# florasion/D-VQVAE

Measured on AMD Instinct MI355X. Metric: grasps/sec at batch=65536, N=1024 pts, K=512, higher is better.
Workload: dtype f32 (GEMMs: every fp32 operand as two fp16 pieces, a1 = fp16(a), a2 = fp16((a - a1) * 2^11), weights pre-scaled by one power of two per output row; the 3 partial products a1 b1, a1 b2, a2 b1 are exact in fp32 and accumulate in TWO fp32 accumulators (large / cross terms) on v_mfma_f32_16x16x32_f16; d

## Files before the change

d-vqvae_amd/csrc/pointnet_filter.hip:

```cpp
#include "dvq_internal.h"
#include "pn_filter.h"
#include <vector>

namespace {

typedef __bf16 qbf16x8 __attribute__((ext_vector_type(8)));
typedef _Float16 qf16x8 __attribute__((ext_vector_type(8)));
typedef _Float16 qf16x2 __attribute__((ext_vector_type(2)));
typedef float qf32x2 __attribute__((ext_vector_type(2)));

constexpr float C_ID = 5.0e-5f;
constexpr float DELTA = 1.0e-6f;
constexpr float NEG_BIG = -3.0e38f;

constexpr int F_STAGE2 = 2 * 64 * 128;
constexpr int IMG_OFF_TI = 1024 * 256, IMG_OFF_WN = IMG_OFF_TI + 4096, IMG_OFF_RN = IMG_OFF_WN + 4096;
constexpr int IMG_OFF_W2 = IMG_OFF_RN + 4096, IMG_OFF_K2 = IMG_OFF_W2 + 2 * 128 * 128, IMG_BYTES = IMG_OFF_K2 + 512;
constexpr int F_STAGE3 = 64 * 256;
constexpr int F_OFF_TB = 2 * F_STAGE3;
constexpr int F_SLOT = 4 * 2 * 2 * 2 * 64;
constexpr int F_OFF_W1 = F_OFF_TB + 8 * 4 * 4 * 64 * 4;
constexpr int F_OFF_B1 = F_OFF_W1 + 64 * 4 * 4;
constexpr int F_OFF_B2 = F_OFF_B1 + 64 * 4;
constexpr int F_OFF_K2 = F_OFF_B2 + 128 * 4;
constexpr int F_OFF_SC = F_OFF_K2 + 128 * 4;
constexpr int F_OFF_TI = F_OFF_SC + 64;
constexpr int F_OFF_CS = F_OFF_TI + 4096;
constexpr int F_OFF_WS = F_OFF_CS + 512;
constexpr int F_OFF_E2 = F_OFF_WS + 64;
constexpr int F_LDS = F_OFF_E2 + 4096;
constexpr int F_LDS_TAIL = F_LDS + 3 * 4096 + 4 * 512;
static_assert(F_OFF_W1 >= 2 * F_STAGE2, "the conv3 stages and the triple buffer cover the W2 region");

__device__ __forceinline__ float max_nc(float a, float b) { return __builtin_amdgcn_fmed3f(a, b, 3.0e38f); }
__device__ __forceinline__ float min_nc(float a, float b) { return __builtin_amdgcn_fmed3f(a, b, NEG_BIG); }

__device__ __forceinline__ void q_split2(const float (&v)[8], float s, qf16x8& p1, qf16x8& p2) {
    unsigned hb[4], lb[4];
#pragma unroll
    for (int j = 0; j < 4; ++j) {
        const float a0 = v[2 * j], a1 = v[2 * j + 1];
        asm("v_fma_mixlo_f16 %0, %1, %2, 0 op_sel:[0,0,0] op_sel_hi:[0,0,0]" : "=v"(hb[j]) : "v"(a0), "v"(s));
        asm("v_fma_mixhi_f16 %0, %1, %2, 0 op_sel:[0,0,0] op_sel_hi:[0,0,0]" : "+v"(hb[j]) : "v"(a1), "v"(s));
        asm("v_fma_mixlo_f16 %0, %1, %2, -%3 op_sel:[0,0,0] op_sel_hi:[0,0,1]" : "=v"(lb[j]) : "v"(a0), "v"(s), "v"(hb[j]));
        asm("v_fma_mixhi_f16 %0, %1, %2, -%3 op_sel:[0,0,1] op_sel_hi:[0,0,1]" : "+v"(lb[j]) : "v"(a1), "v"(s), "v"(hb[j]));
    }
    p1 = __builtin_bit_cast(qf16x8, uint4{hb[0], hb[1], hb[2], hb[3]});
    p2 = __builtin_bit_cast(qf16x8, uint4{lb[0], lb[1], lb[2], lb[3]});
}

__device__ __forceinline__ void w2_issue(const uint16_t* __restrict__ planes, int row0, char* stage, int wave, int lane) {
#pragma unroll
    for (int i = 0; i < 4; ++i) {
        const int id = wave * 4 + i;
        const int pl = id >> 3, rb = id & 7;
        const int row = rb * 8 + (lane >> 3);
        const uint16_t* src = planes + pl * (128L * 64) + (long)(row0 + row) * 64 + 8 * ((lane & 7) ^ ((row >> 1) & 7));
        __builtin_amdgcn_global_load_lds((const __attribute__((address_space(1))) void*)src,
                                         (__attribute__((address_space(3))) void*)(stage + (pl * 64 + rb * 8) * 128), 16, 0, 0);
    }
}
__device__ __forceinline__ qf16x8 w2_frag(const char* stage, int pl, int row, int chunk) {
    return *reinterpret_cast<const qf16x8*>(stage + (pl * 64 + row) * 128 + 16 * (chunk ^ ((row >> 1) & 7)));
}

struct W3Regs { uint4 a, b, c, d; };
__device__ __forceinline__ const uint4* w3_src(const char* __restrict__ w3h, int ch0, int wave, int lane, int i) {
    const char* base = w3h + (long)(ch0 + (wave * 4 + i) * 4) * 256;
    const unsigned off = (unsigned)(lane >> 4) * 256u + 16u * (unsigned)(lane & 15);
    return reinterpret_cast<const uint4*>(base + off);
}
__device__ __forceinline__ W3Regs w3_load(const char* __restrict__ w3h, int ch0, int wave, int lane) {
    W3Regs v;
    v.a = *w3_src(w3h, ch0, wave, lane, 0);
    v.b = *w3_src(w3h, ch0, wave, lane, 1);
    v.c = *w3_src(w3h, ch0, wave, lane, 2);
    v.d = *w3_src(w3h, ch0, wave, lane, 3);
    return v;
}
__device__ __forceinline__ uint4* w3_dst(char* stage, int wave, int lane, int i) {
    const int row = (wave * 4 + i) * 4 + (lane >> 4);
    return reinterpret_cast<uint4*>(stage + row * 256 + 16 * ((lane & 15) ^ (row & 15)));
}
__device__ __forceinline__ void w3_store(char* stage, int wave, int lane, const W3Regs& v) {
    *w3_dst(stage, wave, lane, 0) = v.a;
    *w3_dst(stage, wave, lane, 1) = v.b;
    *w3_dst(stage, wave, lane, 2) = v.c;
    *w3_dst(stage, wave, lane, 3) = v.d;
}
__device__ __forceinline__ qf16x8 w3_frag(const char* stage, int row, int chunk) {
    return *reinterpret_cast<const qf16x8*>(stage + row * 256 + 16 * (chunk ^ (row & 15)));
}

__device__ __forceinline__ void merge3(float& a1, float& a2, float& a3, float b1, float b2, float b3) {
    const float x = min_nc(a1, b1), y = max_nc(a2, b2), z = min_nc(a2, b2), w = max_nc(a3, b3);
    a1 = max_nc(a1, b1);
    a2 = max_nc(x, y);
    a3 = max_nc(min_nc(x, y), max_nc(z, w));
}

__device__ __forceinline__ float wave_max(float v) {
#pragma unroll
    for (int o = 32; o >= 1; o >>= 1) v = fmaxf(v, __shfl_xor(v, o));
    return v;
}


__device__ __forceinline__ float g_half_sum(float v) {
    const auto r = __builtin_amdgcn_permlane32_swap(__float_as_uint(v), __float_as_uint(v), false, false);
    return __uint_as_float(r[0]) + __uint_as_float(r[1]);
}
__device__ __forceinline__ float g_half_max(float v) {
    const auto r = __builtin_amdgcn_permlane32_swap(__float_as_uint(v), __float_as_uint(v), false, false);
    return fmaxf(__uint_as_float(r[0]), __uint_as_float(r[1]));
}
template <int CTRL>
__device__ __forceinline__ float g_dpp(float v) {
    return __builtin_bit_cast(float, __builtin_amdgcn_update_dpp(0, __builtin_bit_cast(int, v), CTRL, 0xf, 0xf, true));
}
__device__ __forceinline__ float g_wave_max(float v) {
    v = fmaxf(v, g_dpp<0xB1>(v));
    v = fmaxf(v, g_dpp<0x4E>(v));
    v = fmaxf(v, g_dpp<0x141>(v));
    v = fmaxf(v, g_dpp<0x140>(v));
    v = g_half_max(v);
    return fmaxf(__int_as_float(__builtin_amdgcn_readlane(__float_as_int(v), 0)), __int_as_float(__builtin_amdgcn_readlane(__float_as_int(v), 16)));
}
__device__ __forceinline__ float g_wave_sum(float v) {
    v += g_dpp<0xB1>(v);
    v += g_dpp<0x4E>(v);
    v += g_dpp<0x141>(v);
    v += g_dpp<0x140>(v);
    v = g_half_sum(v);
    return __int_as_float(__builtin_amdgcn_readlane(__float_as_int(v), 0)) + __int_as_float(__builtin_amdgcn_readlane(__float_as_int(v), 16));
}
template <int C>
__device__ __forceinline__ void pn_point_in(const float* __restrict__ src, int N, const float* __restrict__ t, float (&x)[4]) {
    float x0 = src[0], x1 = src[N], x2 = src[2L * N];
    const float x3 = (C > 3) ? src[3L * N] : 0.f;
    if (t) {
        const float n0 = fmaf(x2, t[6], fmaf(x1, t[3], x0 * t[0]));
        const float n1 = fmaf(x2, t[7], fmaf(x1, t[4], x0 * t[1]));
        const float n2 = fmaf(x2, t[8], fmaf(x1, t[5], x0 * t[2]));
        x0 = n0; x1 = n1; x2 = n2;
    }
    x[0] = x0; x[1] = x1; x[2] = x2; x[3] = x3;
}

template <int C>
__device__ __forceinline__ void pn_conv1_split(const float (&xin)[4], const float* w1s, const float* b1s, int h_op, qf16x8 (&h1a)[4], qf16x8 (&h1b)[4],
                                               float& r_p_out) {
    float v[4][8];
    float amax = 0.f;
#pragma unroll
    for (int s = 0; s < 4; ++s) {
#pragma unroll
        for (int j = 0; j < 8; ++j) {
            const f32x4 w = *reinterpret_cast<const f32x4*>(w1s + 32 * h_op + 64 * s + 4 * j);
            float a = fmaf(xin[0], w[0], (b1s + 8 * h_op)[16 * s + j]);
            a = fmaf(xin[1], w[1], a);
            a = fmaf(xin[2], w[2], a);
            if constexpr (C > 3) a = fmaf(xin[3], w[3], a);
            v[s][j] = fmaxf(a, 0.f);
        }
#pragma unroll
        for (int j = 0; j < 8; j += 2) amax = fmaxf(fmaxf(amax, v[s][j]), v[s][j + 1]);
    }
    amax = g_half_max(amax);
    float s_p = 1.f, r_p = 1.f;
    {
        const int ex = (int)((__float_as_uint(amax) >> 23) & 255u);
        if (ex > 20 && ex < 235) {
            s_p = __uint_as_float((unsigned)(127 + 15 - (ex - 126)) << 23);
            r_p = __uint_as_float((unsigned)(127 - 15 + (ex - 126)) << 23);
        }
    }
#pragma unroll
    for (int s = 0; s < 4; ++s) q_split2(v[s], s_p, h1a[s], h1b[s]);
    r_p_out = r_p;
}
template <class Frag, class Emit>
__device__ __forceinline__ void pn_conv2_block(const qf16x8 (&h1a)[4], const qf16x8 (&h1b)[4], float r_p, int t4, const float* k2s, const float* b2s,
                                               int h_op, Frag frag, Emit emit) {
    {
        f32x16 acc;
#pragma unroll
        for (int e = 0; e < 16; ++e) acc[e] = 0.f;
        qf16x8 w1f[4];
#pragma unroll
        for (int s = 0; s < 4; ++s) {
            w1f[s] = frag(t4, 0, s);
            const qf16x8 w2f = frag(t4, 1, s);
            acc = __builtin_amdgcn_mfma_f32_32x32x16_f16(w2f, h1a[s], acc, 0, 0, 0);
            acc = __builtin_amdgcn_mfma_f32_32x32x16_f16(w1f[s], h1b[s], acc, 0, 0, 0);
        }
#pragma unroll
        for (int s = 0; s < 4; ++s) acc = __builtin_amdgcn_mfma_f32_32x32x16_f16(w1f[s], h1a[s], acc, 0, 0, 0);
        float o[16];
#pragma unroll
        for (int e = 0; e < 16; ++e) {
            const int ch = 32 * t4 + (e & 3) + 8 * (e >> 2);
            o[e] = fmaxf(fmaf(acc[e] * r_p, (k2s + 4 * h_op)[ch], (b2s + 4 * h_op)[ch]), 0.f);
        }
        emit(t4, o);
    }
}
template <int C, class Frag, class Emit>
__device__ __forceinline__ void pn_conv12_block(const float (&xin)[4], const float* w1s, const float* b1s, const float* k2s, const float* b2s,
                                                int h_op, Frag frag, Emit emit) {
    qf16x8 h1a[4], h1b[4];
    float r_p;
    pn_conv1_split<C>(xin, w1s, b1s, h_op, h1a, h1b, r_p);
#pragma unroll
    for (int t4 = 0; t4 < 4; ++t4) pn_conv2_block(h1a, h1b, r_p, t4, k2s, b2s, h_op, frag, emit);
}
__device__ __forceinline__ void pn_store_row16(float* dst, const float (&o)[16]) {
#pragma unroll
    for (int g = 0; g < 4; ++g) *reinterpret_cast<f32x4*>(dst + 8 * g) = f32x4{o[4 * g], o[4 * g + 1], o[4 * g + 2], o[4 * g + 3]};
}

template <int C, bool TAIL>
__global__ __launch_bounds__(256, 2) void pn_trunk_filter_kernel(const float* __restrict__ pc, const float* __restrict__ trans,
                                                                 int N, int Npad, int tiles, int deal, long B, const float* __restrict__ W1,
                                                                 const float* __restrict__ b1,
                                                                 const float* __restrict__ b2, const char* __restrict__ w3f,
                                                                 float* __restrict__ h2buf, f32x4* __restrict__ part, qf32x2* __restrict__ part2,
                                                                 unsigned* __restrict__ tstat, const float* __restrict__ cbuf,
                                                                 int abl_arg ) {
    const int abl = DVQ_DIAG_ON ? abl_arg : 0;
    extern __shared__ __attribute__((aligned(16))) char fl[];
    float* tb = reinterpret_cast<float*>(fl + F_OFF_TB);
    float* w1s = reinterpret_cast<float*>(fl + F_OFF_W1);
    float* b1s = reinterpret_cast<float*>(fl + F_OFF_B1);
    float* b2s = reinterpret_cast<float*>(fl + F_OFF_B2);
    float* scs = reinterpret_cast<float*>(fl + F_OFF_SC);
    float* tis = reinterpret_cast<float*>(fl + F_OFF_TI);
    float* wst = reinterpret_cast<float*>(fl + F_OFF_WS);
    const int tid = threadIdx.x, lane = tid & 63;
    const int wave = __builtin_amdgcn_readfirstlane(tid >> 6);
    const int r = lane & 31, h = lane >> 5;
    int h_op = h;
    asm("" : "+v"(h_op));
    constexpr int NPB = TAIL ? 1 : 2;
    const long b_raw = TAIL ? (long)blockIdx.x * 4 + wave : (long)(blockIdx.x / deal);
    const bool live = !TAIL || b_raw < B;
    const long b = live ? b_raw : B - 1;
    const int tile = TAIL ? deal : (int)(blockIdx.x % deal);
    const long rec = b * tiles + tile;
    float* cs = reinterpret_cast<float*>(fl + (TAIL ? F_LDS + 3 * 4096 + 512 * wave : F_OFF_CS));
    float* e2s = reinterpret_cast<float*>(fl + F_OFF_E2) + (TAIL ? 1024 * wave : 0);

    const unsigned long long t_start = (abl & PN_ABL_STAMPS) ? __builtin_amdgcn_s_memtime() : 0ull;
    const unsigned long long r_start = (abl & PN_ABL_CLOCK) ? __builtin_amdgcn_s_memrealtime() : 0ull;
    unsigned long long t_a = 0, t_b = 0, t_c = 0;
    const uint16_t* w2pl = reinterpret_cast<const uint16_t*>(w3f + IMG_OFF_W2);
    w2_issue(w2pl, 0, fl, wave, lane);
    w2_issue(w2pl, 64, fl + F_STAGE2, wave, lane);
    float* k2s = reinterpret_cast<float*>(fl + F_OFF_K2);
    if (tid < 128) k2s[tid] = reinterpret_cast<const float*>(w3f + IMG_OFF_K2)[tid];
    w1s[tid] = W1[tid];
    if (tid < 64) b1s[tid] = b1[tid];
    if (tid < 128) b2s[tid] = b2[tid];
    *reinterpret_cast<f32x4*>(tis + 4 * tid) = *reinterpret_cast<const f32x4*>(w3f + IMG_OFF_TI + 16 * tid);
    if (TAIL) { cs[lane] = cbuf[b * 128 + lane]; cs[64 + lane] = cbuf[b * 128 + 64 + lane]; }
    else if (tid < 128) cs[tid] = cbuf[b * 128 + tid];

    float xin[NPB][4];
    int pidx[NPB];
    bool badpt = false;
#pragma unroll
    for (int pb = 0; pb < NPB; ++pb) {
        int p = point_of_slot(tile, TAIL ? r : wave * 64 + pb * 32 + r, deal);
        pidx[pb] = p;
        if (p >= N) p %= N;
        pn_point_in<C>(pc + b * (long)C * N + p, N, trans ? trans + b * 9 : nullptr, xin[pb]);
        const float x0 = xin[pb][0], x1 = xin[pb][1], x2 = xin[pb][2], x3 = xin[pb][3];
        badpt = badpt || !(fabsf(x0) < 3.0e38f) || !(fabsf(x1) < 3.0e38f) || !(fabsf(x2) < 3.0e38f) || !(fabsf(x3) < 3.0e38f);
    }
    dvq_dma_barrier();
    __builtin_amdgcn_s_waitcnt(0x0F70);
    if (abl & PN_ABL_STAMPS) t_a = __builtin_amdgcn_s_memtime();
    float cnorm;
    {
        const float cq = fmaf(cs[lane], cs[lane], cs[64 + lane] * cs[64 + lane]);
        cnorm = sqrtf(g_wave_sum(cq)) * 1.0001f;
    }

// ... 267 lines not shown
            F_INTERLEAVE();
            finish(c, 1, m1, m2);
            F_MFMA_BLOCK(accB, wf[3]);
            F_CHAIN_BLOCK(accA, m1, m2, ctag_c);
            F_INTERLEAVE();
            finish(c, 2, m1, m2);
            F_CHAIN_BLOCK(accB, m1, m2, ctag_c);
            finish(c, 3, m1, m2);
            if (c + 1 < 16) w3_store(fl + (stage ^ 1) * F_STAGE3, wave, lane, wreg);
            stage ^= 1;
        }
    } else {
    f32x4 accP[NRB];
#pragma unroll 1
    for (int c4 = 0; c4 < ((abl & PN_ABL_NO_CONV3) ? 0 : 16); c4 += 4) {
    unsigned ctag4[16];
#pragma unroll
    for (int e = 0; e < 16; ++e) asm("s_or_b32 %0, %1, %2" : "=s"(ctag4[e]) : "s"((unsigned)(((c4 >> 2) & 3) << 5)), "i"(e));
#pragma unroll
    for (int u = 0; u < 4; ++u) {
        const int c = c4 + u;
        const int stage = u & 1;
        const bool pending = u != 0;
        if (!(abl & PN_ABL_NO_CHUNK_BARRIER)) dvq_lds_barrier();
        if (c + 1 < 16 && !(abl & PN_ABL_NO_W3_LOADS)) wreg = w3_load(w3h, 64 * (c + 1), wave, lane);
        if (u == 0 && c > 0 && !(abl & PN_ABL_NO_PUBLISH)) {
            publish(c - 4 + wave);
            dvq_lds_barrier();
        }
        const char* st = fl + stage * F_STAGE3;
        qf16x8 wf[4][4];
#pragma unroll
        for (int cb = 0; cb < 4; ++cb)
#pragma unroll
            for (int ks = 0; ks < 4; ++ks) wf[cb][ks] = w3_frag(st, 16 * cb + l16, 4 * ks + qchunk);
        f32x4 accA[NRB], accB[NRB];
        float m1, m2;
        F_MFMA_BLOCK(accA, wf[0]);
        if (pending) {
            F_CHAIN_BLOCK(accP, m1, m2, ctag4);
            F_INTERLEAVE();
            if (!(abl & PN_ABL_NO_HANDOVER)) finish(c - 1, 3, m1, m2);
            else if (m1 + m2 == 12345.f) tb[lane] = m1;
        }
        F_MFMA_BLOCK(accB, wf[1]);
        F_CHAIN_BLOCK(accA, m1, m2, ctag4);
        F_INTERLEAVE();
        if (!(abl & PN_ABL_NO_HANDOVER)) finish(c, 0, m1, m2);
        else if (m1 + m2 == 12345.f) tb[lane] = m1;
        F_MFMA_BLOCK(accA, wf[2]);
        F_CHAIN_BLOCK(accB, m1, m2, ctag4);
        F_INTERLEAVE();
        if (!(abl & PN_ABL_NO_HANDOVER)) finish(c, 1, m1, m2);
        else if (m1 + m2 == 12345.f) tb[lane] = m1;
        F_MFMA_BLOCK(accP, wf[3]);
        F_CHAIN_BLOCK(accA, m1, m2, ctag4);
        F_INTERLEAVE();
        if (!(abl & PN_ABL_NO_HANDOVER)) finish(c, 2, m1, m2);
        else if (m1 + m2 == 12345.f) tb[lane] = m1;
        if (u == 3) {
            F_CHAIN_BLOCK(accP, m1, m2, ctag4);
            if (!(abl & PN_ABL_NO_HANDOVER)) finish(c, 3, m1, m2);
            else if (m1 + m2 == 12345.f) tb[lane] = m1;
        }
        if (c + 1 < 16 && !(abl & PN_ABL_NO_W3_LOADS)) w3_store(fl + (stage ^ 1) * F_STAGE3, wave, lane, wreg);
    }
    }
    }
#undef F_MFMA_BLOCK
#undef F_CHAIN_BLOCK
#undef F_INTERLEAVE
    dvq_lds_barrier();
    if constexpr (TAIL) {
#pragma unroll 1
        for (int q = 12; q < 16; ++q) publish(q);
    } else if (!(abl & PN_ABL_NO_PUBLISH)) {
        publish(12 + wave);
    }
    if ((abl & PN_ABL_STAMPS) && tid == 0) {
        const unsigned long long t_end = __builtin_amdgcn_s_memtime();
        auto q = [](unsigned long long d) { d >>= 6; return (unsigned)(d > 255 ? 255 : d); };
        tstat[4 * rec + 3] = q(t_a - t_start) | (q(t_b - t_a) << 8) | (q(t_c - t_b) << 16) | (q((t_end - t_c) >> 3) << 24);
        if (abl & PN_ABL_CLOCK) {
            const unsigned long long r_end = __builtin_amdgcn_s_memrealtime();
            tstat[4 * rec + 3] = (unsigned)((t_end - t_start) * 100ull / (r_end - r_start + 1));
        }
    }
}

template <int CTRL>
__device__ __forceinline__ float q_dpp(float v) {
    return __builtin_bit_cast(float, __builtin_amdgcn_update_dpp(0, __builtin_bit_cast(int, v), CTRL, 0xf, 0xf, true));
}
__device__ __forceinline__ float exact_dot_regs(const f32x4& w0, const f32x4& w1, const f32x4& a, const f32x4& c) {
    float s = w0[0] * a[0];
    s = fmaf(w0[1], a[1], s);
    s = fmaf(w0[2], a[2], s);
    s = fmaf(w0[3], a[3], s);
    s = fmaf(w1[0], c[0], s);
    s = fmaf(w1[1], c[1], s);
    s = fmaf(w1[2], c[2], s);
    s = fmaf(w1[3], c[3], s);
    s += q_dpp<0xB1>(s);
    s += q_dpp<0x4E>(s);
    s += q_dpp<0x141>(s);
    s += q_dpp<0x140>(s);
    return s;
}
__device__ __forceinline__ float exact_dot(const f32x4& w0, const f32x4& w1, const float* __restrict__ hrow, int j) {
    return exact_dot_regs(w0, w1, *reinterpret_cast<const f32x4*>(hrow + 4 * j), *reinterpret_cast<const f32x4*>(hrow + 4 * j + 64));
}
__device__ __forceinline__ float max_nan(float a, float b) { return (a != a || b != b) ? __builtin_nanf("") : fmaxf(a, b); }

__device__ __forceinline__ unsigned f2key(float v) {
    const unsigned u = __float_as_uint(v);
    return (u & 0x80000000u) ? ~u : (u | 0x80000000u);
}
__device__ __forceinline__ float key2f(unsigned k) { return __uint_as_float((k & 0x80000000u) ? (k & 0x7fffffffu) : ~k); }

__device__ unsigned long long g_pn_faults[2];

constexpr int PAIR_CAP = 2048;
constexpr int FB_CAP = 512;
constexpr unsigned short NO_ANCHOR = 0xFFFFu;
constexpr int TODO_CAP = 2 * PAIR_CAP;
template <int C>
__global__ __launch_bounds__(256, 4) void pn_exact_kernel(const f32x4* __restrict__ part, const qf32x2* __restrict__ part2, int tiles, int deal,
                                                       float* h2buf , int recompute,
                                                       const float* __restrict__ pc, const float* __restrict__ trans,
                                                       const float* __restrict__ W1, const float* __restrict__ b1, const float* __restrict__ b2,
                                                       const char* __restrict__ w3f,
                                                       int N, int Npad, const float* __restrict__ w3, const float* __restrict__ b3,
                                                       const float* __restrict__ wnorm, const float* __restrict__ rnorm,
                                                       const unsigned* __restrict__ tstat, const float* __restrict__ cbuf, int relu, int exhaustive,
                                                       int pair_cap, int fb_cap, float* __restrict__ feat, long ld_feat,
                                                       unsigned long long* __restrict__ stats, int abl_arg) {
    const int abl = DVQ_DIAG_ON ? abl_arg : 0;
    __shared__ unsigned short anchor[1024];
    __shared__ int pair_list[PAIR_CAP];
    __shared__ int fb_list[FB_CAP];
    __shared__ short all_list[1024];
    __shared__ int pair_count, fb_count, all_count;
    __shared__ float fb_part[4][16];
    __shared__ float hm[PN_MAX_TILES], dm[PN_MAX_TILES], rd[PN_MAX_TILES];
    __shared__ unsigned best_k[1024];
    __shared__ float wcs[1024];
    __shared__ int pcnt[1024];
    __shared__ unsigned sorted[PAIR_CAP];
    __shared__ int wave_tot[4];
    __shared__ unsigned row_mask[32];
    __shared__ unsigned done_mask[PN_MAX_POINTS / 32];
    __shared__ int todo_count;
    __shared__ __attribute__((aligned(16))) float w1s[64 * 4 + 64];
    static_assert(PAIR_CAP >= 1024, "sorted[] holds the 1 024 anchors");
    static_assert(PN_MAX_POINTS <= 65536, "a point fits a 16-bit list entry");
    const int tid = threadIdx.x, g = tid >> 4, j = tid & 15;
    const long b = blockIdx.x;
    if (tid == 0) { pair_count = 0; fb_count = 0; all_count = 0; todo_count = 0; }
    if (tid < 32) row_mask[tid] = 0;
    done_mask[tid] = 0; done_mask[tid + 256] = 0;
    w1s[tid] = W1[tid];
    if (tid < 64) w1s[256 + tid] = b1[tid];
#pragma unroll
    for (int i = 0; i < 4; ++i) pcnt[tid + 256 * i] = 0;
    int nonfinite_point = 0;
    if (tid < tiles) {
        const unsigned* ts = tstat + 4 * (b * tiles + tid);
        hm[tid] = __uint_as_float(ts[0]) * 1.00001f;
        dm[tid] = __uint_as_float(ts[1]) * 1.00001f;
        rd[tid] = __uint_as_float(ts[2]) * 1.00001f;
        nonfinite_point = ts[3] != 0 && !(abl & PN_ABL_STAMPS);
    }
    if (__syncthreads_or(nonfinite_point)) {
        for (int n = tid; n < 1024; n += 256) feat[b * ld_feat + n] = __builtin_nanf("");
        return;
    }
    float* h2 = h2buf + b * (long)Npad * 128;
    const bool wrap_small = Npad <= 2 * N;
    const f32x4* pt = part + b * (long)tiles * 1024;
    const qf32x2* pt2 = part2 + b * (long)tiles * 1024;
    const bool stamps = DVQ_DIAG_ON && stats && (abl & PN_ABL_STAMPS);
    unsigned long long tp[8] = {0, 0, 0, 0, 0, 0, 0, 0};
    if (stamps) tp[0] = __builtin_amdgcn_s_memtime();
    unsigned n_single = 0, n_multi = 0, n_cand = 0, n_wave = 0, n_suspect = 0;
    auto bound_of = [&](float wn, float rn, int t) { return fmaf(rn, dm[t], fmaf(wn, rd[t], fmaf(C_ID * wn, dm[t], 2.0f * DELTA * wn * hm[t]))); };
    struct Scan { float lb, ub, e_all, top_star; int t_star; bool all; };
    auto scan_tiles = [&](int n, float wn, float rn, float top0, float top1, float top2, float top3) {
        Scan s;
        bool nonfinite = false;
        auto fold = [&](int t, float top) {
            const float e = bound_of(wn, rn, t), l = top - e;
            nonfinite = nonfinite || !(e < 3.0e38f) || !(fabsf(top) < 3.0e38f);
            s.e_all = fmaxf(s.e_all, e);
            if (l > s.lb) { s.t_star = t; s.top_star = top; }
            s.lb = fmaxf(s.lb, l);
            s.ub = fmaxf(s.ub, top + e);
        };
        {
            const float e0 = bound_of(wn, rn, 0);
            s.e_all = e0;
            s.lb = top0 - e0;
            s.ub = top0 + e0;
            s.t_star = 0;
            s.top_star = top0;
            nonfinite = !(e0 < 3.0e38f) || !(fabsf(top0) < 3.0e38f);
            if (tiles > 1) fold(1, top1);
            if (tiles > 2) fold(2, top2);
            if (tiles > 3) fold(3, top3);
        }
        for (int t0 = 4; t0 < tiles; t0 += 4) {
            float top[4];
#pragma unroll
            for (int u = 0; u < 4; ++u) top[u] = pt[min(t0 + u, tiles - 1) * 1024 + n][0];
#pragma unroll
            for (int u = 0; u < 4; ++u)
                if (t0 + u < tiles) fold(t0 + u, top[u]);
        }
        s.all = exhaustive || nonfinite || !(s.e_all < 3.0e38f) || !(s.lb > NEG_BIG) || !(s.lb < 3.0e38f);
        return s;
    };
    auto point_of_score = [&](int t, float v) {
        int p = point_of_slot(t, slot_of_id(__float_as_uint(v) & 255u), deal);
        if (p >= N) p = wrap_small ? p - N : p % N;
        if (abl & PN_ABL_FEW_ROWS) p &= 63;
        return p;
    };
    unsigned short* todo = reinterpret_cast<unsigned short*>(pair_list);
    int todo_base = 0;
    auto claim = [&](int p) {
        const unsigned bit = 1u << (p & 31);
        if (atomicOr(&done_mask[p >> 5], bit) & bit) return;
        const int slot = atomicAdd(&todo_count, 1) - todo_base;
        if (slot < TODO_CAP) todo[slot] = (unsigned short)p;
    };
    auto fill_rows = [&](bool all) {
        dvq_lds_barrier();
        const int end = __builtin_amdgcn_readfirstlane(todo_count), listed = end - todo_base;
        todo_base = end;
        const bool forced = listed > TODO_CAP;
        const bool whole = all || forced;
        const int cnt = whole ? N : listed;
        const int lane = tid & 63, r = lane & 31, h = lane >> 5;
        const float* k2g = reinterpret_cast<const float*>(w3f + IMG_OFF_K2);
        const uint16_t* w2pl = reinterpret_cast<const uint16_t*>(w3f + IMG_OFF_W2);
        for (int i0 = 32 * __builtin_amdgcn_readfirstlane(tid >> 6); i0 < cnt; i0 += 128) {
            if (whole && !forced && done_mask[i0 >> 5] == ~0u) continue;
            int h_op = h;
            asm volatile("" : "+v"(h_op));
            const int i = min(i0 + r, cnt - 1);
            const int p = whole ? i : (int)todo[i];
            float x[4];
            pn_point_in<C>(pc + b * (long)C * N + p, N, trans ? trans + b * 9 : nullptr, x);
            float* row = h2 + (long)p * 128 + 4 * h;
            const bool mine = i0 + r < cnt;
            qf16x8 h1a[4], h1b[4];
            float r_p;
            pn_conv1_split<C>(x, w1s, w1s + 256, h_op, h1a, h1b, r_p);
#pragma unroll 1
            for (int t4 = 0; t4 < 4; ++t4)
                pn_conv2_block(h1a, h1b, r_p, t4, k2g, b2, h_op,
                               [&](int t, int pl, int s) { return *reinterpret_cast<const qf16x8*>(w2pl + pl * (128 * 64) + (32 * t + r) * 64 + 8 * (2 * s + h)); },
                               [&](int t, const float (&o)[16]) { if (mine) pn_store_row16(row + 32 * t, o); });
            if (whole && lane == 0) done_mask[i0 >> 5] = ~0u;
            if (stats && lane == 0) {
                atomicAdd(stats + 10, 1ull);
                atomicAdd(stats + 11, (unsigned long long)min(32, cnt - i0));
            }
        }
        asm volatile("s_waitcnt vmcnt(0)" ::: "memory");
        dvq_lds_barrier();
    };
    auto sort_by_point = [&](auto code_at, int count, bool first) {
        for (int i = tid; i < count; i += 256) {
            const unsigned code = code_at(i);
            if (code != ~0u) atomicAdd(&pcnt[(code >> 10) & 1023], 1);
        }
        dvq_lds_barrier();
        const int c0 = pcnt[4 * tid], c1 = pcnt[4 * tid + 1], c2 = pcnt[4 * tid + 2], c3 = pcnt[4 * tid + 3];
        if (stats) {
            const unsigned m = (unsigned)(c0 != 0) | (unsigned)(c1 != 0) << 1 | (unsigned)(c2 != 0) << 2 | (unsigned)(c3 != 0) << 3;
            const int sh = 4 * (tid & 7);
            int rows;
            if (first) { if (m) atomicOr(&row_mask[tid >> 3], m << sh); rows = __popc(m); }
            else rows = __popc(m & ~(row_mask[tid >> 3] >> sh));
            if (rows) atomicAdd(stats + 8, (unsigned long long)rows);
        }
        int incl = c0 + c1 + c2 + c3;
        int lane_op = tid & 63;
        asm volatile("" : "+v"(lane_op));
#pragma unroll
        for (int o = 1; o < 64; o <<= 1) {
            const int v = __builtin_amdgcn_ds_bpermute(4 * (lane_op - o), incl);
            if ((tid & 63) >= o) incl += v;
        }
        if ((tid & 63) == 63) wave_tot[tid >> 6] = incl;
        dvq_lds_barrier();
        int base = 0;
        for (int w = 0; w < (tid >> 6); ++w) base += wave_tot[w];
        const int total = wave_tot[0] + wave_tot[1] + wave_tot[2] + wave_tot[3];
        const int excl = base + incl - (c0 + c1 + c2 + c3);
        pcnt[4 * tid] = excl;
        pcnt[4 * tid + 1] = excl + c0;
        pcnt[4 * tid + 2] = excl + c0 + c1;
        pcnt[4 * tid + 3] = excl + c0 + c1 + c2;
        dvq_lds_barrier();
        for (int i = tid; i < count; i += 256) {
            const unsigned code = code_at(i);
            if (code != ~0u) sorted[atomicAdd(&pcnt[(code >> 10) & 1023], 1)] = code;
        }
        dvq_lds_barrier();
        return total;
    };
    auto dots = [&](int total, bool first) {
        const int per = (total + 15) >> 4, i0 = g * per, i1 = min(total, i0 + per);
        f32x4 cen_a = {0.f, 0.f, 0.f, 0.f}, cen_b = cen_a;
        if (first) { cen_a = *reinterpret_cast<const f32x4*>(cbuf + b * 128 + 4 * j); cen_b = *reinterpret_cast<const f32x4*>(cbuf + b * 128 + 4 * j + 64); }
        for (int i = i0; i < i1; i += 4) {
            f32x4 w0[4], w1[4], ha[4], hb[4];
            int nn[4];
#pragma unroll
            for (int u = 0; u < 4; ++u) {
                const unsigned code = sorted[min(i + u, i1 - 1)];
                nn[u] = (int)(code & 1023u);
                const unsigned woff = (code & 1023u) * 512u + 16u * (unsigned)j, hoff = (code >> 10) * 512u + 16u * (unsigned)j;
                w0[u] = *reinterpret_cast<const f32x4*>(reinterpret_cast<const char*>(w3) + woff);
                w1[u] = *reinterpret_cast<const f32x4*>(reinterpret_cast<const char*>(w3) + woff + 256);
                ha[u] = *reinterpret_cast<const f32x4*>(reinterpret_cast<const char*>(h2) + hoff);
                hb[u] = *reinterpret_cast<const f32x4*>(reinterpret_cast<const char*>(h2) + hoff + 256);
            }
            float v[4], wc[4];
#pragma unroll
            for (int u = 0; u < 4; ++u) {
                v[u] = exact_dot_regs(w0[u], w1[u], ha[u], hb[u]);
                wc[u] = first ? exact_dot_regs(w0[u], w1[u], cen_a, cen_b) : 0.f;
            }
            if (j == 0) {
#pragma unroll
                for (int u = 0; u < 4; ++u)
                    if (i + u < i1) {
                        if (first) { best_k[nn[u]] = f2key(v[u]); wcs[nn[u]] = wc[u]; }
                        else atomicMax(&best_k[nn[u]], f2key(v[u]));
                    }
            }
        }
    };
    {
        float top[4][4], wn[4], rn[4];
#pragma unroll
        for (int ci = 0; ci < 4; ++ci) {
            const int n = tid + 256 * ci;
#pragma unroll
            for (int u = 0; u < 4; ++u) top[ci][u] = pt[min(u, tiles - 1) * 1024 + n][0];
            wn[ci] = wnorm[n]; rn[ci] = rnorm[n];
        }
#pragma unroll
        for (int ci = 0; ci < 4; ++ci) {
            const int n = tid + 256 * ci;
            const Scan s = scan_tiles(n, wn[ci], rn[ci], top[ci][0], top[ci][1], top[ci][2], top[ci][3]);
            best_k[n] = f2key(NEG_BIG);
            wcs[n] = 0.f;
            if (s.all) {
                all_list[atomicAdd(&all_count, 1)] = (short)n;
                anchor[n] = NO_ANCHOR;
            } else
                anchor[n] = (unsigned short)point_of_score(s.t_star, s.top_star);
        }
    }
    dvq_lds_barrier();
    if (stamps) tp[1] = __builtin_amdgcn_s_memtime();
    auto anchor_code = [&](int n) { const unsigned p = anchor[n]; return p == NO_ANCHOR ? ~0u : (unsigned)n | (p << 10); };
    const int n_anchor = sort_by_point(anchor_code, 1024, true);
#pragma unroll
    for (int i = 0; i < 4; ++i) pcnt[tid + 256 * i] = 0;
    if (stamps) tp[2] = __builtin_amdgcn_s_memtime();
    if (recompute) {
        for (int i = tid; i < n_anchor; i += 256) {
            const int p = (int)(sorted[i] >> 10);
            if (i == 0 || (int)(sorted[i - 1] >> 10) != p) claim(p);
        }
        fill_rows(false);
    }
    if (!(abl & PN_ABL_NO_DOTS)) dots(n_anchor, true);
    dvq_lds_barrier();
    if (stamps) tp[3] = __builtin_amdgcn_s_memtime();
    float lo_0 = 1.f, lo_1 = 1.f, lo_2 = 1.f, lo_3 = 1.f, hi_0 = 0.f, hi_1 = 0.f, hi_2 = 0.f, hi_3 = 0.f;
    f32x4 nf0 = pt[tid], nf1 = pt[min(1, tiles - 1) * 1024 + tid], nf2 = pt[min(2, tiles - 1) * 1024 + tid], nf3 = pt[min(3, tiles - 1) * 1024 + tid];
    qf32x2 ng0 = pt2[tid], ng1 = pt2[min(1, tiles - 1) * 1024 + tid], ng2 = pt2[min(2, tiles - 1) * 1024 + tid], ng3 = pt2[min(3, tiles - 1) * 1024 + tid];
    float nwn = wnorm[tid], nrn = rnorm[tid];
#pragma unroll 1
    for (int ci = 0; ci < 4; ++ci) {
        const int n = tid + 256 * ci;
        const float wn = nwn, rn = nrn;
        const f32x4 f0 = nf0, f1 = nf1, f2 = nf2, f3 = nf3;
        const qf32x2 g0 = ng0, g1 = ng1, g2 = ng2, g3 = ng3;
        if (ci < 3) {
            const int nx = n + 256;
            nf0 = pt[nx]; nf1 = pt[min(1, tiles - 1) * 1024 + nx]; nf2 = pt[min(2, tiles - 1) * 1024 + nx]; nf3 = pt[min(3, tiles - 1) * 1024 + nx];
            ng0 = pt2[nx]; ng1 = pt2[min(1, tiles - 1) * 1024 + nx]; ng2 = pt2[min(2, tiles - 1) * 1024 + nx]; ng3 = pt2[min(3, tiles - 1) * 1024 + nx];
            nwn = wnorm[nx]; nrn = rnorm[nx];
        }
        const Scan s = scan_tiles(n, wn, rn, f0[0], f1[0], f2[0], f3[0]);
        if (s.all) continue;
        const float lb = s.lb;
        float L = lb;
        if (!(abl & PN_ABL_NO_RULE2)) {
            const float v1 = key2f(best_k[n]), wc1 = wcs[n];
            L = fmaxf(lb, (v1 - wc1) - 4.0e-7f * (fabsf(v1) + fabsf(wc1)));
        }
        int cands = 1;
        bool whole = false;
        float lo_c = lb, hi_c = s.ub;
        auto consider = [&](int t, const f32x4& q, const qf32x2& q45) {
            const float et = bound_of(wn, rn, t);
            const unsigned suspect = (__float_as_uint(q[3]) >> 16) & 1u;
            n_suspect += suspect;
            if (!suspect && !(q[0] + et >= L)) return;
            unsigned flags = __float_as_uint(q[3]) & 0xFFFFu;
            unsigned forced = suspect ? 0xFFFFu : 0u;
            auto take = [&](float v) {
                const int p = point_of_score(t, v);
                const int slot = atomicAdd(&pair_count, 1);
                if (slot < pair_cap) pair_list[slot] = n | (p << 10);
                else {
                    const unsigned bit = 1u << pn_group_of_id(__float_as_uint(v));
                    flags |= bit;
                    forced |= bit;
                }
                ++cands;
            };
            const float sc5[5] = {q[0], q[1], q[2], q45[0], q45[1]};
#pragma unroll 1
            for (int k = (t == s.t_star ? 1 : 0); k < 5; ++k) {
                const float v = k == 0 ? sc5[0] : k == 1 ? sc5[1] : k == 2 ? sc5[2] : k == 3 ? sc5[3] : sc5[4];
                if (!(v + et >= L)) break;
                take(v);
            }
            while (flags) {
                const int wh = __ffs(flags) - 1;
                flags &= flags - 1;
                if (!((forced >> wh) & 1u) && !(abl & PN_ABL_NO_RULE1)) {
                    auto of_group = [&](float v) { return pn_group_of_id(__float_as_uint(v)) == wh; };
                    const bool m0 = of_group(sc5[0]), m1 = of_group(sc5[1]), m2 = of_group(sc5[2]), m3 = of_group(sc5[3]), m4 = of_group(sc5[4]);
                    const float second = m4 ? sc5[4] : m3 ? sc5[3] : m2 ? sc5[2] : m1 ? sc5[1] : sc5[0];
                    const float u = (int)m0 + (int)m1 + (int)m2 + (int)m3 + (int)m4 >= 2 ? second : sc5[4];
                    if (u + et < L) continue;
                }
                const int slot = atomicAdd(&fb_count, 1);
                if (slot < fb_cap) fb_list[slot] = n | (t << 10) | (wh << 20);
                else if (!whole) {
                    whole = true;
                    all_list[atomicAdd(&all_count, 1)] = (short)n;
                }
                ++n_wave;
            }
        };
        f32x4 q0 = f0, q1 = f1, q2 = f2, q3 = f3;
        qf32x2 h0 = g0, h1 = g1, h2q = g2, h3 = g3;
#pragma unroll 1
        for (int t0 = 0; t0 < tiles; t0 += 4) {
            if (t0 > 0) {
                q0 = pt[min(t0, tiles - 1) * 1024 + n]; q1 = pt[min(t0 + 1, tiles - 1) * 1024 + n];
                q2 = pt[min(t0 + 2, tiles - 1) * 1024 + n]; q3 = pt[min(t0 + 3, tiles - 1) * 1024 + n];
                h0 = pt2[min(t0, tiles - 1) * 1024 + n]; h1 = pt2[min(t0 + 1, tiles - 1) * 1024 + n];
                h2q = pt2[min(t0 + 2, tiles - 1) * 1024 + n]; h3 = pt2[min(t0 + 3, tiles - 1) * 1024 + n];
            }
#pragma unroll 1
            for (int u = 0; u < 4 && t0 + u < tiles; ++u) {
                const f32x4 q = u == 0 ? q0 : u == 1 ? q1 : u == 2 ? q2 : q3;
                const qf32x2 q45 = u == 0 ? h0 : u == 1 ? h1 : u == 2 ? h2q : h3;
                consider(t0 + u, q, q45);
            }
        }
        if (whole) { lo_c = 1.f; hi_c = 0.f; }
        lo_0 = ci == 0 ? lo_c : lo_0; hi_0 = ci == 0 ? hi_c : hi_0;
        lo_1 = ci == 1 ? lo_c : lo_1; hi_1 = ci == 1 ? hi_c : hi_1;
        lo_2 = ci == 2 ? lo_c : lo_2; hi_2 = ci == 2 ? hi_c : hi_2;
        lo_3 = ci == 3 ? lo_c : lo_3; hi_3 = ci == 3 ? hi_c : hi_3;
        n_single += cands == 1;
        n_multi += cands != 1;
        n_cand += cands;
    }
    dvq_lds_barrier();
    if (stamps) tp[4] = __builtin_amdgcn_s_memtime();
    auto eval_all_list = [&](int count) {
        for (int i = 0; i < count; i += 4) {
            f32x4 w0[4], w1[4];
            float best[4];
#pragma unroll
            for (int u = 0; u < 4; ++u) {
                const int n = all_list[min(i + u, count - 1)];
                w0[u] = *reinterpret_cast<const f32x4*>(w3 + n * 128 + 4 * j);
                w1[u] = *reinterpret_cast<const f32x4*>(w3 + n * 128 + 4 * j + 64);
                best[u] = NEG_BIG;
            }
            for (int p = g; p < N; p += 16) {
                const float* hr = reinterpret_cast<const float*>(reinterpret_cast<const char*>(h2) + ((unsigned)p * 512u + 16u * (unsigned)j));
                const f32x4 ha = *reinterpret_cast<const f32x4*>(hr), hb = *reinterpret_cast<const f32x4*>(hr + 64);
#pragma unroll
                for (int u = 0; u < 4; ++u) best[u] = max_nan(best[u], exact_dot_regs(w0[u], w1[u], ha, hb));
                if (best[0] != best[0] && best[1] != best[1] && best[2] != best[2] && best[3] != best[3]) break;
            }
            if (j == 0) {
#pragma unroll
                for (int u = 0; u < 4; ++u) fb_part[u][g] = best[u];
            }
            dvq_lds_barrier();
            if (tid < 4 && i + tid < count) {
                float v = fb_part[tid][0];
                for (int k = 1; k < 16; ++k) v = max_nan(v, fb_part[tid][k]);
                best_k[all_list[i + tid]] = (v != v) ? 0xffffffffu : f2key(v);
            }
            dvq_lds_barrier();
        }
    };
    unsigned n_bad = 0;
    int n_sorted = 0, nfb = 0;
#pragma unroll 1
    for (int pass = 0; pass < 2; ++pass) {
        if (pass == 0) {
            const int npairs = min(pair_count, pair_cap);
            n_sorted = sort_by_point([&](int i) { return (unsigned)pair_list[i]; }, npairs, false);
            if (stamps) tp[5] = __builtin_amdgcn_s_memtime();
            nfb = (abl & PN_ABL_NO_GROUPS) ? 0 : min(fb_count, fb_cap);
            if (recompute && all_count == 0) {
                for (int i = tid; i < n_sorted; i += 256) {
                    const int p = (int)(sorted[i] >> 10);
                    if (i == 0 || (int)(sorted[i - 1] >> 10) != p) claim(p);
                }
                for (int i = tid; i < 16 * nfb; i += 256) {
                    const int code = fb_list[i >> 4];
                    int p = point_of_slot((code >> 10) & 1023, pn_group_slot((code >> 20) & 15, i & 15), deal);
                    if (p >= N) p %= N;
                    claim(p);
                }
            }
        } else {
            dvq_lds_barrier();
            if (tid == 0) all_count = 0;
            dvq_lds_barrier();
#pragma unroll
            for (int ci = 0; ci < 4; ++ci) {
                const int n = tid + 256 * ci;
                const float lo_c = ci == 0 ? lo_0 : ci == 1 ? lo_1 : ci == 2 ? lo_2 : lo_3, hi_c = ci == 0 ? hi_0 : ci == 1 ? hi_1 : ci == 2 ? hi_2 : hi_3;
                if (!(lo_c <= hi_c) || (abl & ~PN_ABL_VALID)) continue;
                const float v = key2f(best_k[n]), wc = wcs[n];
                const float x = v - wc, slack = 4.0e-7f * (fabsf(v) + fabsf(wc));
                if (!(x >= lo_c - slack && x <= hi_c + slack)) {
                    all_list[atomicAdd(&all_count, 1)] = (short)n;
                    ++n_bad;
                }
            }
            dvq_lds_barrier();
        }
        const int n_all = __builtin_amdgcn_readfirstlane(all_count);
        if (recompute && (pass == 0 || n_all > 0)) fill_rows(n_all > 0);
        if (pass == 0) {
            if (!(abl & PN_ABL_NO_DOTS)) dots(n_sorted, false);
            if (stamps) tp[6] = __builtin_amdgcn_s_memtime();
            for (int i = tid >> 6; i < nfb; i += 4) {
                const int code = fb_list[i];
                const int n = code & 1023, t = (code >> 10) & 1023, grp = (code >> 20) & 15;
                const float* wr = reinterpret_cast<const float*>(reinterpret_cast<const char*>(w3) + ((unsigned)n * 512u + 16u * (unsigned)j));
                const f32x4 w0 = *reinterpret_cast<const f32x4*>(wr), w1 = *reinterpret_cast<const f32x4*>(wr + 64);
                float best = NEG_BIG;
                {
                    f32x4 ha[4], hb[4];
#pragma unroll
                    for (int u = 0; u < 4; ++u) {
                        int p = point_of_slot(t, pn_group_slot(grp, 4 * (g & 3) + u), deal);
                        if (p >= N) p %= N;
                        const float* hr = reinterpret_cast<const float*>(reinterpret_cast<const char*>(h2) + ((unsigned)p * 512u + 16u * (unsigned)j));
                        ha[u] = *reinterpret_cast<const f32x4*>(hr);
                        hb[u] = *reinterpret_cast<const f32x4*>(hr + 64);
                    }
#pragma unroll
                    for (int u = 0; u < 4; ++u) best = fmaxf(best, exact_dot_regs(w0, w1, ha[u], hb[u]));
                }
                if (j == 0) atomicMax(&best_k[n], f2key(best));
            }
            dvq_lds_barrier();
        }
        eval_all_list(n_all);
    }
    if (n_suspect) atomicAdd(&g_pn_faults[0], (unsigned long long)n_suspect);
    if (n_bad) atomicAdd(&g_pn_faults[1], (unsigned long long)n_bad);
    int tid_op = tid;
    asm volatile("" : "+v"(tid_op));
#pragma unroll
    for (int i = 0; i < 4; ++i) {
        const int n = tid_op + 256 * i;
        const unsigned k = best_k[n];
        const float v = (k == 0xffffffffu ? __builtin_nanf("") : key2f(k)) + b3[n];
        feat[b * ld_feat + n] = relu ? (v != v ? v : fmaxf(v, 0.f)) : v;
    }
    if (stamps && tid == 0) {
        const unsigned long long t_end = __builtin_amdgcn_s_memtime();
        atomicAdd(stats + 4, (tp[1] - tp[0]) + (tp[4] - tp[3])); atomicAdd(stats + 5, (tp[2] - tp[1]) + (tp[5] - tp[4]));
        atomicAdd(stats + 6, (tp[3] - tp[2]) + (tp[6] - tp[5])); atomicAdd(stats + 7, t_end - tp[6]);
        atomicAdd(stats + 9, tp[3] - tp[0]);
    }
    if (stats) {
        if (n_single) atomicAdd(stats + 0, (unsigned long long)n_single);
        if (n_multi) atomicAdd(stats + 1, (unsigned long long)n_multi);
        if (n_wave) atomicAdd(stats + 2, (unsigned long long)n_wave);
        if (n_cand) atomicAdd(stats + 3, (unsigned long long)n_cand);
    }
}

constexpr int CENTER_SPB = 4;
template <int C>
__global__ __launch_bounds__(256) void pn_center_kernel(const float* __restrict__ pc, const float* __restrict__ trans, int N, long B,
                                                        const float* __restrict__ W1, const float* __restrict__ b1,
                                                        const float* __restrict__ W2, const float* __restrict__ b2,
                                                        float* __restrict__ cbuf, unsigned* __restrict__ tstat, int tiles) {
    __shared__ float w2t[64][129];
    __shared__ float h1c[4][64];
    __shared__ float h2c[4][128];
    const int tid = threadIdx.x, q = tid >> 6, k = tid & 63;
    for (int i = tid; i < 128 * 64; i += 256) w2t[i & 63][i >> 6] = W2[i];
    for (int sb = 0; sb < CENTER_SPB; ++sb) {
        const long b = (long)blockIdx.x * CENTER_SPB + sb;
        if (b >= B) break;
        for (int i = tid; i < 4 * tiles; i += 256) tstat[b * 4 * tiles + i] = 0u;
        {
            const int p = (int)(((long)q * N) / 4);
            const float* src = pc + b * (long)C * N + p;
            float x0 = src[0], x1 = src[N], x2 = src[2L * N];
            const float x3 = (C > 3) ? src[3L * N] : 0.f;
            if (trans) {
                const float* t = trans + b * 9;
                const float n0 = fmaf(x2, t[6], fmaf(x1, t[3], x0 * t[0]));
                const float n1 = fmaf(x2, t[7], fmaf(x1, t[4], x0 * t[1]));
                const float n2 = fmaf(x2, t[8], fmaf(x1, t[5], x0 * t[2]));
                x0 = n0; x1 = n1; x2 = n2;
            }
            const float* w = W1 + 4 * k;
            float a = x0 * w[0];
            a = fmaf(x1, w[1], a);
            a = fmaf(x2, w[2], a);
            a = fmaf(x3, w[3], a);
            h1c[q][k] = fmaxf(a + b1[k], 0.f);
        }
        dvq_lds_barrier();
#pragma unroll
        for (int half = 0; half < 2; ++half) {
            const int ch = k + 64 * half;
            float a = 0.f;
            for (int i = 0; i < 64; ++i) a = fmaf(w2t[i][ch], h1c[q][i], a);
            h2c[q][ch] = fmaxf(a + b2[ch], 0.f);
        }
        dvq_lds_barrier();
        if (tid < 128) cbuf[b * 128 + tid] = 0.25f * ((h2c[0][tid] + h2c[1][tid]) + (h2c[2][tid] + h2c[3][tid]));
    }
}

__global__ __launch_bounds__(256) void pn_filter_pack_kernel(const float* __restrict__ w3, _Float16* __restrict__ wh,
                                                             float* __restrict__ tinv, float* __restrict__ wnorm,
                                                             float* __restrict__ rnorm) {
    const int lane = threadIdx.x & 63;
    const int n = blockIdx.x * 4 + (threadIdx.x >> 6);
    const float a = w3[n * 128 + lane], c = w3[n * 128 + 64 + lane];
    const float amax = wave_max(fmaxf(fabsf(a), fabsf(c)));
    float sq = fmaf(a, a, c * c);
#pragma unroll
    for (int o = 32; o >= 1; o >>= 1) sq += __shfl_xor(sq, o);
    float t = 1.f;
    const int ex = (int)((__float_as_uint(amax) >> 23) & 255u);
    if (ex > 20 && ex < 235) t = __uint_as_float((unsigned)(127 + 15 - (ex - 126)) << 23);
    float rs = 0.f;
#pragma unroll
    for (int half = 0; half < 2; ++half) {
        const int pos = 64 * half + lane;
        const int q = pos & 15;
        const int k = (pos & ~15) + ((q & 3) | ((q & 4) << 1) | ((q & 8) >> 1));
        const float v = w3[n * 128 + k] * t;
        const _Float16 hv = (_Float16)v;
        wh[n * 128 + pos] = hv;
        const float res = v - (float)hv;
        rs = fmaf(res, res, rs);
    }
#pragma unroll
    for (int o = 32; o >= 1; o >>= 1) rs += __shfl_xor(rs, o);
    if (lane == 0) {
        tinv[n] = 1.0f / t;
        wnorm[n] = sqrtf(sq) * 1.00001f;
        rnorm[n] = sqrtf(rs) / t * 1.00001f;
    }
}

__global__ __launch_bounds__(256) void pn_filter_pack_w2_kernel(const float* __restrict__ w2, _Float16* __restrict__ planes,
                                                                float* __restrict__ kinv) {
    const int lane = threadIdx.x & 63;
    const int n = blockIdx.x * 4 + (threadIdx.x >> 6);
    const float v = w2[n * 64 + lane];
    const float amax = wave_max(fabsf(v));
    float t = 1.f;
    const int ex = (int)((__float_as_uint(amax) >> 23) & 255u);
    if (ex > 20 && ex < 235) t = __uint_as_float((unsigned)(127 + 15 - (ex - 126)) << 23);
    const float vs = v * t;
    const _Float16 p1 = (_Float16)vs;
    const _Float16 p2 = (_Float16)(vs - (float)p1);
    planes[n * 64 + lane] = p1;
    planes[128 * 64 + n * 64 + lane] = p2;
    if (lane == 0) kinv[n] = 1.0f / t;
}

}

size_t dvq_pn_filter_image_bytes() { return (size_t)IMG_BYTES; }

int dvq_launch_pn_filter_pack(const float* w2, const float* w3, void* image, hipStream_t st) {
    char* im = (char*)image;
    DVQ_LAUNCH(pn_filter_pack_kernel, dim3(256), dim3(256), 0, st, w3, reinterpret_cast<_Float16*>(im),
               reinterpret_cast<float*>(im + IMG_OFF_TI), reinterpret_cast<float*>(im + IMG_OFF_WN),
               reinterpret_cast<float*>(im + IMG_OFF_RN));
    DVQ_CHECK_LAUNCH("pn_filter_pack");
    DVQ_LAUNCH(pn_filter_pack_w2_kernel, dim3(32), dim3(256), 0, st, w2, reinterpret_cast<_Float16*>(im + IMG_OFF_W2),
               reinterpret_cast<float*>(im + IMG_OFF_K2));
    DVQ_CHECK_LAUNCH("pn_filter_pack_w2");
    return DVQ_OK;
}

static int filter_geometry(int N, PnGeometry* g) {
    *g = pn_geometry(N, dvq_knobs().pn_tail != 0);
    DVQ_REQUIRE(g->tiles <= PN_MAX_TILES, "pointnet: the filtered trunk takes at most %d points", PN_MAX_POINTS);
    return DVQ_OK;
}
#ifdef DVQ_DIAG
static int pn_abl() { const char* e = getenv("DVQ_PN_ABL"); return e ? atoi(e) : 0; }
#else
static constexpr int pn_abl() { return 0; }
#endif

using TrunkFilterKernel = decltype(&pn_trunk_filter_kernel<3, false>);
static TrunkFilterKernel trunk_filter_kernel(int C, bool tail) {
    static const TrunkFilterKernel k[2][2] = {{&pn_trunk_filter_kernel<3, false>, &pn_trunk_filter_kernel<3, true>},
                                              {&pn_trunk_filter_kernel<4, false>, &pn_trunk_filter_kernel<4, true>}};
    return k[C == 4][tail];
}
static decltype(&pn_center_kernel<3>) center_kernel(int C) { return C == 4 ? &pn_center_kernel<4> : &pn_center_kernel<3>; }
static decltype(&pn_exact_kernel<3>) exact_kernel(int C) { return C == 4 ? &pn_exact_kernel<4> : &pn_exact_kernel<3>; }
static bool pn_recompute() { return dvq_knobs().pn_recompute && !dvq_knobs().pn_exhaustive; }

int dvq_launch_pn_filter_front(const PnBatch& in, const PnTrunkWeights& w, const PnSlot& sl, unsigned long long* stats, hipStream_t st) {
    PnGeometry g;
    DVQ_PROPAGATE(filter_geometry(in.N, &g));
    static DvqOncePerDevice attr_once[2][2];
    for (int c = 0; c < 2; ++c)
        for (int tail = 0; tail < 2; ++tail)
            DVQ_PROPAGATE(dvq_lds_limit(attr_once[c][tail], reinterpret_cast<const void*>(trunk_filter_kernel(3 + c, tail)),
                                        tail ? F_LDS_TAIL : (DVQ_DIAG_ON ? 100 * 1024 : F_LDS), "pointnet"));
    const long B = in.B, grid = B * g.deal;
    DVQ_REQUIRE(B * g.tiles < (1L << 31), "pointnet: grid too large");
    if (stats && hipMemsetAsync(stats, 0, PN_STATS_BYTES, st) != hipSuccess) {
        dvq_set_error("pointnet: hipMemsetAsync failed");
        return DVQ_ELAUNCH;
    }
    {
// ... 111 lines not shown
```

Before: 191,300.

## Restructure fill_rows: per-wave output column slice with register-resident W2 and prefetched points

The row-filling loop changes from each wave computing all 128 output channels for its own 32 points to each wave computing one 32-channel slice for every point. This lets the wave keep its W2 fragments in registers for the whole loop instead of reloading them from global memory. The next batch of point coordinates is prefetched while the current batch runs its convolution. The transform matrix and the k2/b2 vectors are hoisted into scalars or LDS, done_mask updates are batched to the end of the loop, and the stats and fault atomics move earlier to shorten live ranges. In exchange, every wave now walks all points, so the conv1 work is repeated across the four waves, and register pressure rises.

```diff
diff --git a/d-vqvae_amd/csrc/pointnet_filter.hip b/d-vqvae_amd/csrc/pointnet_filter.hip
--- a/d-vqvae_amd/csrc/pointnet_filter.hip
+++ b/d-vqvae_amd/csrc/pointnet_filter.hip
@@ -133,6 +133,17 @@
     v += g_dpp<0x140>(v);
     v = g_half_sum(v);
     return __int_as_float(__builtin_amdgcn_readlane(__float_as_int(v), 0)) + __int_as_float(__builtin_amdgcn_readlane(__float_as_int(v), 16));
+}
+template <int C>
+__device__ __forceinline__ void pn_point_raw(const float* __restrict__ src, int N, float (&x)[4]) {
+    x[0] = src[0]; x[1] = src[N]; x[2] = src[2L * N];
+    x[3] = (C > 3) ? src[3L * N] : 0.f;
+}
+__device__ __forceinline__ void pn_point_xform(const float (&t)[9], float (&x)[4]) {
+    const float n0 = fmaf(x[2], t[6], fmaf(x[1], t[3], x[0] * t[0]));
+    const float n1 = fmaf(x[2], t[7], fmaf(x[1], t[4], x[0] * t[1]));
+    const float n2 = fmaf(x[2], t[8], fmaf(x[1], t[5], x[0] * t[2]));
+    x[0] = n0; x[1] = n1; x[2] = n2;
 }
 template <int C>
 __device__ __forceinline__ void pn_point_in(const float* __restrict__ src, int N, const float* __restrict__ t, float (&x)[4]) {
@@ -706,15 +717,18 @@
     __shared__ unsigned done_mask[PN_MAX_POINTS / 32];
     __shared__ int todo_count;
     __shared__ __attribute__((aligned(16))) float w1s[64 * 4 + 64];
+    __shared__ float k2s[128], b2s[128];
     static_assert(PAIR_CAP >= 1024, "sorted[] holds the 1 024 anchors");
     static_assert(PN_MAX_POINTS <= 65536, "a point fits a 16-bit list entry");
-    const int tid = threadIdx.x, g = tid >> 4, j = tid & 15;
+    int tid = threadIdx.x;
+    const int g = tid >> 4, j = tid & 15;
     const long b = blockIdx.x;
     if (tid == 0) { pair_count = 0; fb_count = 0; all_count = 0; todo_count = 0; }
     if (tid < 32) row_mask[tid] = 0;
     done_mask[tid] = 0; done_mask[tid + 256] = 0;
     w1s[tid] = W1[tid];
     if (tid < 64) w1s[256 + tid] = b1[tid];
+    if (tid < 128) { k2s[tid] = reinterpret_cast<const float*>(w3f + IMG_OFF_K2)[tid]; b2s[tid] = b2[tid]; }
 #pragma unroll
     for (int i = 0; i < 4; ++i) pcnt[tid + 256 * i] = 0;
     int nonfinite_point = 0;
@@ -788,41 +802,73 @@
         if (slot < TODO_CAP) todo[slot] = (unsigned short)p;
     };
     auto fill_rows = [&](bool all) {
+        const int lane = tid & 63, r = lane & 31, h = lane >> 5;
+        const int wv = __builtin_amdgcn_readfirstlane(tid >> 6);
+        qf16x8 wf[2][4];
+        {
+            const uint16_t* w2pl = reinterpret_cast<const uint16_t*>(w3f + IMG_OFF_W2) + (32 * wv + r) * 64 + 8 * h;
+#pragma unroll
+            for (int pl = 0; pl < 2; ++pl)
+#pragma unroll
+                for (int s = 0; s < 4; ++s) wf[pl][s] = *reinterpret_cast<const qf16x8*>(w2pl + pl * (128 * 64) + 16 * s);
+        }
+        float tm[9] = {0.f, 0.f, 0.f, 0.f, 0.f, 0.f, 0.f, 0.f, 0.f};
+        if (trans) {
+#pragma unroll
+            for (int k = 0; k < 9; ++k) tm[k] = trans[b * 9 + k];
+        }
         dvq_lds_barrier();
+#pragma unroll
+        for (int s = 0; s < 4; ++s) asm volatile("" : "+v"(wf[0][s]), "+v"(wf[1][s]));
+#pragma unroll
+        for (int k = 0; k < 9; ++k) tm[k] = __int_as_float(__builtin_amdgcn_readfirstlane(__float_as_int(tm[k])));
         const int end = __builtin_amdgcn_readfirstlane(todo_count), listed = end - todo_base;
         todo_base = end;
         const bool forced = listed > TODO_CAP;
         const bool whole = all || forced;
         const int cnt = whole ? N : listed;
-        const int lane = tid & 63, r = lane & 31, h = lane >> 5;
-        const float* k2g = reinterpret_cast<const float*>(w3f + IMG_OFF_K2);
-        const uint16_t* w2pl = reinterpret_cast<const uint16_t*>(w3f + IMG_OFF_W2);
-        for (int i0 = 32 * __builtin_amdgcn_readfirstlane(tid >> 6); i0 < cnt; i0 += 128) {
-            if (whole && !forced && done_mask[i0 >> 5] == ~0u) continue;
+        auto next_batch = [&](int i0) {
+            if (whole && !forced)
+                while (i0 < cnt && __builtin_amdgcn_readfirstlane(done_mask[i0 >> 5]) == ~0u) i0 += 32;
+            return i0;
+        };
+        auto request = [&](int i0, int& p, float (&x)[4]) {
+            const int i = min(i0 + r, cnt - 1);
+            p = whole ? i : (int)todo[i];
+            pn_point_raw<C>(pc + b * (long)C * N + p, N, x);
+        };
+        int i0 = next_batch(0), p_next = 0;
+        float x_next[4] = {0.f, 0.f, 0.f, 0.f};
+        if (i0 < cnt) {
+            request(i0, p_next, x_next);
+            asm volatile("" : "+v"(x_next[0]), "+v"(x_next[1]), "+v"(x_next[2]), "+v"(x_next[3]));
+        }
+        while (i0 < cnt) {
+            const int p = p_next;
+            float x[4] = {x_next[0], x_next[1], x_next[2], x_next[3]};
+            if (trans) pn_point_xform(tm, x);
+            const int i1 = next_batch(i0 + 32);
+            if (i1 < cnt) request(i1, p_next, x_next);
             int h_op = h;
             asm volatile("" : "+v"(h_op));
-            const int i = min(i0 + r, cnt - 1);
-            const int p = whole ? i : (int)todo[i];
-            float x[4];
-            pn_point_in<C>(pc + b * (long)C * N + p, N, trans ? trans + b * 9 : nullptr, x);
-            float* row = h2 + (long)p * 128 + 4 * h;
-            const bool mine = i0 + r < cnt;
+            float* row = reinterpret_cast<float*>(reinterpret_cast<char*>(h2) + ((unsigned)p * 512u + 16u * (unsigned)h));
             qf16x8 h1a[4], h1b[4];
             float r_p;
             pn_conv1_split<C>(x, w1s, w1s + 256, h_op, h1a, h1b, r_p);
-#pragma unroll 1
-            for (int t4 = 0; t4 < 4; ++t4)
-                pn_conv2_block(h1a, h1b, r_p, t4, k2g, b2, h_op,
-                               [&](int t, int pl, int s) { return *reinterpret_cast<const qf16x8*>(w2pl + pl * (128 * 64) + (32 * t + r) * 64 + 8 * (2 * s + h)); },
-                               [&](int t, const float (&o)[16]) { if (mine) pn_store_row16(row + 32 * t, o); });
-            if (whole && lane == 0) done_mask[i0 >> 5] = ~0u;
-            if (stats && lane == 0) {
+            pn_conv2_block(h1a, h1b, r_p, wv, k2s, b2s, h_op,
+                           [&](int, int pl, int s) { return wf[pl][s]; },
+                           [&](int t, const float (&o)[16]) { pn_store_row16(row + 32 * t, o); });
+            if (i1 < cnt) asm volatile("" : "+v"(x_next[0]), "+v"(x_next[1]), "+v"(x_next[2]), "+v"(x_next[3]));
+            if (stats && wv == 0 && lane == 0) {
                 atomicAdd(stats + 10, 1ull);
                 atomicAdd(stats + 11, (unsigned long long)min(32, cnt - i0));
             }
+            i0 = i1;
         }
         asm volatile("s_waitcnt vmcnt(0)" ::: "memory");
         dvq_lds_barrier();
+        if (whole)
+            for (int i = tid; i < (N + 31) >> 5; i += 256) done_mask[i] = ~0u;
     };
     auto sort_by_point = [&](auto code_at, int count, bool first) {
         for (int i = tid; i < count; i += 256) {
@@ -1036,6 +1082,13 @@
     }
     dvq_lds_barrier();
     if (stamps) tp[4] = __builtin_amdgcn_s_memtime();
+    if (n_suspect) atomicAdd(&g_pn_faults[0], (unsigned long long)n_suspect);
+    if (stats) {
+        if (n_single) atomicAdd(stats + 0, (unsigned long long)n_single);
+        if (n_multi) atomicAdd(stats + 1, (unsigned long long)n_multi);
+        if (n_wave) atomicAdd(stats + 2, (unsigned long long)n_wave);
+        if (n_cand) atomicAdd(stats + 3, (unsigned long long)n_cand);
+    }
     auto eval_all_list = [&](int count) {
         for (int i = 0; i < count; i += 4) {
             f32x4 w0[4], w1[4];
@@ -1067,10 +1120,10 @@
             dvq_lds_barrier();
         }
     };
-    unsigned n_bad = 0;
     int n_sorted = 0, nfb = 0;
 #pragma unroll 1
     for (int pass = 0; pass < 2; ++pass) {
+        asm volatile("" : "+v"(tid));
         if (pass == 0) {
             const int npairs = min(pair_count, pair_cap);
             n_sorted = sort_by_point([&](int i) { return (unsigned)pair_list[i]; }, npairs, false);
@@ -1092,6 +1145,7 @@
             dvq_lds_barrier();
             if (tid == 0) all_count = 0;
             dvq_lds_barrier();
+            unsigned n_bad = 0;
 #pragma unroll
             for (int ci = 0; ci < 4; ++ci) {
                 const int n = tid + 256 * ci;
@@ -1104,6 +1158,7 @@
                     ++n_bad;
                 }
             }
+            if (n_bad) atomicAdd(&g_pn_faults[1], (unsigned long long)n_bad);
             dvq_lds_barrier();
         }
         const int n_all = __builtin_amdgcn_readfirstlane(all_count);
@@ -1136,8 +1191,6 @@
         }
         eval_all_list(n_all);
     }
-    if (n_suspect) atomicAdd(&g_pn_faults[0], (unsigned long long)n_suspect);
-    if (n_bad) atomicAdd(&g_pn_faults[1], (unsigned long long)n_bad);
     int tid_op = tid;
     asm volatile("" : "+v"(tid_op));
 #pragma unroll
@@ -1152,12 +1205,6 @@
         atomicAdd(stats + 4, (tp[1] - tp[0]) + (tp[4] - tp[3])); atomicAdd(stats + 5, (tp[2] - tp[1]) + (tp[5] - tp[4]));
         atomicAdd(stats + 6, (tp[3] - tp[2]) + (tp[6] - tp[5])); atomicAdd(stats + 7, t_end - tp[6]);
         atomicAdd(stats + 9, tp[3] - tp[0]);
-    }
-    if (stats) {
-        if (n_single) atomicAdd(stats + 0, (unsigned long long)n_single);
-        if (n_multi) atomicAdd(stats + 1, (unsigned long long)n_multi);
-        if (n_wave) atomicAdd(stats + 2, (unsigned long long)n_wave);
-        if (n_cand) atomicAdd(stats + 3, (unsigned long long)n_cand);
     }
 }
 
```

After: 192,700, median of 6. No clear change (+0.7%).
